# JaronTu/Multimodal_MVD_Seg

Hardware: AMD Instinct MI355X
Metric: train-step samples/sec on 4-modality 128^3 patches (PlainConvUNet 3d_fullres, fp32) (higher is better)
Workload: dtype f32; 1 GPU; BASELINE configs[1]: PlainConvUNet 3d_fullres 6 stages 31.2M params, 4x128x128x128 patch, 5 classes, fp32, DC+CE deep supervision, SGD-Nesterov+clip; per_gpu_batch=2, global_batch=2, parallelism=dp1, step_launch=one hipGraph replay per step (captured after 3 eager steps)

## Files before the change

include/mvdseg_hip.h:

```cpp
#ifndef MVDSEG_HIP_H
#define MVDSEG_HIP_H
#include <stddef.h>
#include <stdint.h>

#ifdef __cplusplus
extern "C" {
#endif

#define MVD_VERSION 100
#define MVD_MAX_TAPS 27

int mvd_version(void);
const char *mvd_last_error(void);
int mvd_has_mfma(void);
int mvd_set_conv_engine(int mode);
int mvd_set_wino_min_items(long n);

int mvd_pack_weight(const float *w, float *wf, float *wb, int K, int C, int T, int transposed, void *stream);

size_t mvd_conv_fwd_workspace_bytes(int N, long out_voxels, int K);
int mvd_conv3d_fwd(const float *x1, int C1, const float *x2, int C2, const float *wf, const float *bias, float *y,
                   int N, int D, int H, int W, int K, const int ksize[3], const int stride[3], void *ws,
                   size_t ws_bytes, void *stream);
int mvd_conv3d_dgrad(const float *dy, const float *wb, float *dx1, int C1, float *dx2, int C2, int N, int D, int H,
// ... 1 lines not shown
int mvd_conv_wino_applicable(int N, int D, int H, int W, int C1, int C2, int K, const int ksize[3], const int stride[3]);
size_t mvd_wino_weight_elems(int C, int K);
int mvd_wino_mode(void);
int mvd_pack_weight_wino(const float *w, float *uf, float *ub, int K, int C, void *stream);
int mvd_pack_weights_batch(int n, const float *const *w, float *const *wf, float *const *wb, float *const *uf,
                           float *const *ub, const int *K, const int *C, const int *T, const int *transposed,
                           void *stream);
int mvd_conv3d_fwd_wino(const float *x1, int C1, const float *x2, int C2, const float *wf, const float *uf,
                        const float *bias, float *y, int N, int D, int H, int W, int K, const int ksize[3],
                        const int stride[3], void *ws, size_t ws_bytes, void *stream);
size_t mvd_conv_stats_tiles(int D, int H, int W);
int mvd_conv3d_fwd_wino_stats(const float *x1, int C1, const float *x2, int C2, const float *wf, const float *uf,
                              const float *bias, float *y, float *stats, int *stats_done, int N, int D, int H, int W,
                              int K, const int ksize[3], const int stride[3], void *ws, size_t ws_bytes, void *stream);
int mvd_conv3d_dgrad_wino(const float *dy, const float *wb, const float *ub, float *dx1, int C1, float *dx2, int C2, int N,
                          int D, int H, int W, int K, const int ksize[3], const int stride[3], void *ws, size_t ws_bytes,
                          void *stream);
int mvd_set_wino3_min_items(long n);
int mvd_conv_wino3_applicable(int N, int D, int H, int W, int C1, int C2, int K, const int ksize[3], const int stride[3]);
size_t mvd_wino3_weight_elems(int C, int K);
int mvd_pack_weight_wino3(const float *w, float *vf, float *vb, int K, int C, void *stream);
int mvd_pack_weights_batch3(int n, const float *const *w, float *const *wf, float *const *wb, float *const *uf,
                            float *const *ub, float *const *vf, float *const *vb, const int *K, const int *C,
                            const int *T, const int *transposed, void *stream);
int mvd_conv3d_fwd_wino3(const float *x1, int C1, const float *x2, int C2, const float *wf, const float *vf,
                         const float *bias, float *y, int N, int D, int H, int W, int K, const int ksize[3],
                         const int stride[3], void *ws, size_t ws_bytes, void *stream);
int mvd_conv3d_fwd_wino3_stats(const float *x1, int C1, const float *x2, int C2, const float *wf, const float *vf,
                               const float *bias, float *y, float *stats, int *stats_done, int N, int D, int H, int W,
                               int K, const int ksize[3], const int stride[3], void *ws, size_t ws_bytes, void *stream);
int mvd_conv3d_dgrad_wino3(const float *dy, const float *wb, const float *vb, float *dx1, int C1, float *dx2, int C2,
                           int N, int D, int H, int W, int K, const int ksize[3], const int stride[3], void *ws,
                           size_t ws_bytes, void *stream);
size_t mvd_conv3d_wgrad_workspace_bytes(int C, int K, int T, int N, int Do, int Ho, int Wo);
int mvd_conv3d_wgrad(const float *x1, int C1, const float *x2, int C2, const float *dy, float *dw, float *dbias,
                     int N, int D, int H, int W, int K, const int ksize[3], const int stride[3], void *ws,
                     size_t ws_bytes, void *stream);

int mvd_convT3d_fwd(const float *x, const float *wf, const float *bias, float *y, int N, int D, int H, int W, int C,
                    int K, const int stride[3], void *ws, size_t ws_bytes, void *stream);
int mvd_convT3d_dgrad(const float *dy, const float *wb, float *dx, int N, int D, int H, int W, int C, int K,
                      const int stride[3], void *ws, size_t ws_bytes, void *stream);
size_t mvd_convT3d_wgrad_workspace_bytes(int C, int K, int T, int N, int D, int H, int W);
int mvd_convT3d_wgrad(const float *x, const float *dy, float *dw, float *dbias, int N, int D, int H, int W, int C,
                      int K, const int stride[3], void *ws, size_t ws_bytes, void *stream);

int mvd_pack_weight_bf16(const float *w, uint16_t *wf, uint16_t *wb, int K, int C, int T, int transposed, void *stream);
int mvd_pack_weights_bf16_batch(int n, const float *const *w, uint16_t *const *wf, uint16_t *const *wb, const int *K,
                                const int *C, const int *T, const int *transposed, void *stream);
int mvd_conv3d_fwd_bf16(const uint16_t *x1, int C1, const uint16_t *x2, int C2, const uint16_t *wf, const float *bias,
                        uint16_t *y, int N, int D, int H, int W, int K, const int ksize[3], const int stride[3],
                        void *ws, size_t ws_bytes, void *stream);
int mvd_conv3d_dgrad_bf16(const uint16_t *dy, const uint16_t *wb, uint16_t *dx1, int C1, uint16_t *dx2, int C2, int N,
                          int D, int H, int W, int K, const int ksize[3], const int stride[3], void *ws, size_t ws_bytes,
                          void *stream);
int mvd_convT3d_fwd_bf16(const uint16_t *x, const uint16_t *wf, const float *bias, uint16_t *y, int N, int D, int H, int W,
                         int C, int K, const int stride[3], void *ws, size_t ws_bytes, void *stream);
int mvd_convT3d_dgrad_bf16(const uint16_t *dy, const uint16_t *wb, uint16_t *dx, int N, int D, int H, int W, int C, int K,
                           const int stride[3], void *ws, size_t ws_bytes, void *stream);
int mvd_conv3d_wgrad_bf16(const uint16_t *x1, int C1, const uint16_t *x2, int C2, const uint16_t *dy, float *dw,
                          float *dbias, int N, int D, int H, int W, int K, const int ksize[3], const int stride[3],
                          void *ws, size_t ws_bytes, void *stream);
int mvd_convT3d_wgrad_bf16(const uint16_t *x, const uint16_t *dy, float *dw, float *dbias, int N, int D, int H, int W,
                           int C, int K, const int stride[3], void *ws, size_t ws_bytes, void *stream);
int mvd_conv3d_fwd_bf16_stats_tiles(int N, int D, int H, int W, int C1, int C2, int K, const int ksize[3],
                                    const int stride[3]);
// ... 157 lines not shown
```

multimodal_mvd_seg_amd/_lib.py:

```python
import ctypes
import os
from ctypes import c_float, c_int, c_long, c_size_t, c_void_p

_HERE = os.path.dirname(os.path.abspath(__file__))
LIB_PATH = os.path.join(_HERE, "libmvdseg_hip.so")

_P = c_void_p
_I3 = ctypes.c_int * 3

SIGNATURES = {
    "mvd_version": (c_int, []),
    "mvd_last_error": (ctypes.c_char_p, []),
    "mvd_has_mfma": (c_int, []),
    "mvd_set_conv_engine": (c_int, [c_int]),
    "mvd_set_wino_min_items": (c_int, [c_long]),
    "mvd_pack_weight": (c_int, [_P, _P, _P, c_int, c_int, c_int, c_int, _P]),
    "mvd_conv_fwd_workspace_bytes": (c_size_t, [c_int, c_long, c_int]),
    "mvd_conv3d_fwd": (c_int, [_P, c_int, _P, c_int, _P, _P, _P, c_int, c_int, c_int, c_int, c_int, _I3, _I3, _P,
                               c_size_t, _P]),
    "mvd_conv3d_dgrad": (c_int, [_P, _P, _P, c_int, _P, c_int, c_int, c_int, c_int, c_int, c_int, _I3, _I3, _P,
                                 c_size_t, _P]),
    "mvd_conv3d_wgrad_workspace_bytes": (c_size_t, [c_int, c_int, c_int, c_int, c_int, c_int, c_int]),
    "mvd_conv3d_wgrad": (c_int, [_P, c_int, _P, c_int, _P, _P, _P, c_int, c_int, c_int, c_int, c_int, _I3, _I3, _P,
                                 c_size_t, _P]),
    "mvd_convT3d_fwd": (c_int, [_P, _P, _P, _P, c_int, c_int, c_int, c_int, c_int, c_int, _I3, _P, c_size_t, _P]),
    "mvd_convT3d_dgrad": (c_int, [_P, _P, _P, c_int, c_int, c_int, c_int, c_int, c_int, _I3, _P, c_size_t, _P]),
    "mvd_convT3d_wgrad_workspace_bytes": (c_size_t, [c_int, c_int, c_int, c_int, c_int, c_int, c_int]),
    "mvd_convT3d_wgrad": (c_int, [_P, _P, _P, _P, c_int, c_int, c_int, c_int, c_int, c_int, _I3, _P, c_size_t, _P]),
    "mvd_conv_wino_applicable": (c_int, [c_int, c_int, c_int, c_int, c_int, c_int, c_int, _I3, _I3]),
    "mvd_wino_mode": (c_int, []),
    "mvd_wino_weight_elems": (c_size_t, [c_int, c_int]),
    "mvd_pack_weight_wino": (c_int, [_P, _P, _P, c_int, c_int, _P]),
    "mvd_pack_weights_batch": (c_int, [c_int] + [_P] * 9 + [_P]),
    "mvd_conv3d_fwd_wino": (c_int, [_P, c_int, _P, c_int, _P, _P, _P, _P, c_int, c_int, c_int, c_int, c_int, _I3, _I3, _P,
                                    c_size_t, _P]),
    "mvd_conv_stats_tiles": (c_size_t, [c_int, c_int, c_int]),
    "mvd_conv3d_fwd_wino_stats": (c_int, [_P, c_int, _P, c_int, _P, _P, _P, _P, _P, _P, c_int, c_int, c_int, c_int, c_int,
                                          _I3, _I3, _P, c_size_t, _P]),
    "mvd_conv3d_dgrad_wino": (c_int, [_P, _P, _P, _P, c_int, _P, c_int, c_int, c_int, c_int, c_int, c_int, _I3, _I3, _P,
                                      c_size_t, _P]),
    "mvd_set_wino3_min_items": (c_int, [c_long]),
    "mvd_conv_wino3_applicable": (c_int, [c_int, c_int, c_int, c_int, c_int, c_int, c_int, _I3, _I3]),
    "mvd_wino3_weight_elems": (c_size_t, [c_int, c_int]),
    "mvd_pack_weight_wino3": (c_int, [_P, _P, _P, c_int, c_int, _P]),
    "mvd_pack_weights_batch3": (c_int, [c_int] + [_P] * 11 + [_P]),
    "mvd_conv3d_fwd_wino3": (c_int, [_P, c_int, _P, c_int, _P, _P, _P, _P, c_int, c_int, c_int, c_int, c_int, _I3, _I3, _P,
                                     c_size_t, _P]),
    "mvd_conv3d_fwd_wino3_stats": (c_int, [_P, c_int, _P, c_int, _P, _P, _P, _P, _P, _P, c_int, c_int, c_int, c_int, c_int,
                                           _I3, _I3, _P, c_size_t, _P]),
    "mvd_conv3d_dgrad_wino3": (c_int, [_P, _P, _P, _P, c_int, _P, c_int, c_int, c_int, c_int, c_int, c_int, _I3, _I3, _P,
                                       c_size_t, _P]),
    "mvd_conv3d_wgrad_bf16": (c_int, [_P, c_int, _P, c_int, _P, _P, _P, c_int, c_int, c_int, c_int, c_int, _I3, _I3, _P,
                                      c_size_t, _P]),
    "mvd_convT3d_wgrad_bf16": (c_int, [_P, _P, _P, _P, c_int, c_int, c_int, c_int, c_int, c_int, _I3, _P, c_size_t,
                                       _P]),
    "mvd_instnorm_lrelu_fwd_prestats": (c_int, [_P, _P, c_long, _P, _P, _P, _P, _P, c_int, c_long, c_int, c_float, c_float,
                                                _P, c_size_t, _P]),
    "mvd_conv3d_fwd_bf16_stats_tiles": (c_int, [c_int, c_int, c_int, c_int, c_int, c_int, c_int, _I3, _I3]),
    "mvd_set_bf16_zmarch_kernel": (c_int, [c_int]),
    "mvd_set_bf16_wgrad_kernel": (c_int, [c_int]),
    "mvd_conv3d_dgrad_acc_ok": (c_int, [c_int, c_int, c_int, c_int, c_int, c_int, c_int, _I3, _I3]),
    "mvd_conv3d_dgrad_acc": (c_int, [_P, _P, _P, c_int, c_int, c_int, c_int, c_int, c_int, _I3, _I3, _P]),
    "mvd_conv3d_dgrad_bf16_acc": (c_int, [_P, _P, _P, c_int, c_int, c_int, c_int, c_int, c_int, _I3, _I3, _P, c_size_t, _P]),
    "mvd_conv3d_fwd_bf16_prologue_ok": (c_int, [c_int, c_int, c_int, c_int, c_int, c_int, c_int, _I3, _I3]),
    "mvd_conv3d_wgrad_bf16_prologue_ok": (c_int, [c_int, c_int, c_int, c_int, c_int, c_int, c_int, _I3, _I3]),
    "mvd_conv3d_wgrad_bf16_fused": (c_int, [_P, c_int, _P, _P, _P, c_int, c_int, c_int, c_int, c_int, _I3, _I3, _P, _P, c_float,
                                            _P, c_size_t, _P]),
    "mvd_instnorm_stats_bf16": (c_int, [_P, c_int, _P, _P, _P, _P, _P, _P, c_int, c_long, c_int, c_float, _P, c_size_t, _P]),
    "mvd_conv3d_fwd_bf16_fused": (c_int, [_P, c_int, _P, c_int, _P, _P, _P, c_int, c_int, c_int, c_int, c_int, _I3, _I3, _P,
                                          _P, c_float, _P, _P, _P, c_size_t, _P]),
    "mvd_instnorm_finalize_tiles": (c_int, [_P, c_long, _P, _P, _P, _P, _P, _P, c_int, c_long, c_int, c_float, _P]),
    "mvd_instnorm_lrelu_apply_bf16": (c_int, [_P, _P, _P, _P, c_int, c_long, c_int, c_float, _P]),
    "mvd_instnorm_lrelu_fwd_bf16": (c_int, [_P, c_int, _P, _P, _P, _P, _P, c_int, c_long, c_int, c_float, c_float, _P,
                                            c_size_t, _P]),
    "mvd_instnorm_lrelu_bwd_bf16": (c_int, [_P, c_int, _P, _P, _P, _P, _P, _P, _P, _P, c_int, c_long, c_int, c_float, _P,
                                            c_size_t, _P]),
    "mvd_seghead_fwd_bf16": (c_int, [_P, _P, _P, _P, c_int, c_long, c_int, c_int, _P]),
    "mvd_seghead_bwd_bf16": (c_int, [_P, _P, _P, _P, _P, _P, c_int, c_long, c_int, c_int, c_int, _P, c_size_t, _P]),
    "mvd_seghead_bf16_fused_ok": (c_int, [c_int, c_long, c_int, c_int]),
    "mvd_seghead_fwd_fused": (c_int, [_P, _P, _P, _P, _P, c_float, _P, _P, _P, c_int, c_long, c_int, c_int, _P]),
    "mvd_seghead_bwd_fused": (c_int, [_P, _P, _P, _P, _P, c_float, _P, _P, _P, _P, _P, c_int, c_long, c_int, c_int, c_int, _P,
                                      c_size_t, _P]),
    "mvd_instnorm_stats_from_tiles": (c_int, [_P, c_long, _P, _P, c_int, c_long, c_int, c_float, _P, c_size_t, _P]),
    "mvd_seghead_fwd_bf16_fused": (c_int, [_P, _P, _P, c_float, _P, _P, _P, c_int, c_long, c_int, c_int, _P]),
# ... 111 lines not shown
```

multimodal_mvd_seg_amd/csrc/conv.hip:

```cpp
#include "common.h"
#include "conv_geom.h"

namespace mvd {

static int g_engine_mode = 0;
#define g_wino_off (wino_mode() == 0)
static const int g_transp_off = getenv("MVD_TRANSP") ? (atoi(getenv("MVD_TRANSP")) == 0) : 0;
static long g_wino_min_items = getenv("MVD_WINO_MIN") ? atol(getenv("MVD_WINO_MIN")) : 256;
static const long kWino3MinItemsDefault = 128;
static long g_wino3_min_items = getenv("MVD_WINO3_MIN") ? atol(getenv("MVD_WINO3_MIN")) : kWino3MinItemsDefault;
static long wino3_items(int D, int H, int W, int K) { return (long)((D + 3) / 4) * ((H + 7) / 8) * ((W + 7) / 8) * (K / 32); }

__global__ void k_fwd_scalar(FwdGeom g, const float *__restrict__ a1, const float *__restrict__ a2,
                             const float *__restrict__ w, const float *__restrict__ bias, float *__restrict__ y1,
                             float *__restrict__ y2) {
    const int K = g.K1 + g.K2, C = g.C1 + g.C2;
    const int CK = wl_ck(C);
    const long total = (long)g.N * g.Do * g.Ho * g.Wo * K;
    for (long idx = (long)blockIdx.x * blockDim.x + threadIdx.x; idx < total; idx += (long)gridDim.x * blockDim.x) {
        int k = (int)(idx % K);
        long r = idx / K;
        int ow = (int)(r % g.Wo);
        r /= g.Wo;
        int oh = (int)(r % g.Ho);
// ... 562 lines not shown
                            const int st[3]) {
    memset(&g, 0, sizeof(g));
    g.N = N;
    g.Di = D; g.Hi = H; g.Wi = W;
    g.Do = out_dim(D, ks[0], st[0]); g.Ho = out_dim(H, ks[1], st[1]); g.Wo = out_dim(W, ks[2], st[2]);
    g.Db = g.Do; g.Hb = g.Ho; g.Wb = g.Wo;
    g.C1 = C1; g.C2 = C2; g.K = K;
    int t = 0;
    for (int a = 0; a < ks[0]; a++)
        for (int b = 0; b < ks[1]; b++)
            for (int c = 0; c < ks[2]; c++) {
                g.off[t][0] = a - (ks[0] - 1) / 2;
                g.off[t][1] = b - (ks[1] - 1) / 2;
                g.off[t][2] = c - (ks[2] - 1) / 2;
                g.wt[t] = t;
                t++;
            }
    g.ntaps = g.T = t;
    for (int a = 0; a < 3; a++) {
        g.sa[a] = st[a];
        g.sb[a] = 1;
    }
    g.transposed_out = 0;
}

size_t mvd_conv3d_wgrad_workspace_bytes(int C, int K, int T, int N, int Do, int Ho, int Wo) {
    WgradGeom g;
    memset(&g, 0, sizeof(g));
    g.N = N; g.Do = Do; g.Ho = Ho; g.Wo = Wo; g.C1 = C; g.C2 = 0; g.K = K; g.ntaps = g.T = T;
    size_t a = max_sz(wgrad_scalar_ws(g), wgrad_mfma_ws(g));
    return max_sz(a, colsum_ws((long)N * Do * Ho * Wo, K));
}

int mvd_conv3d_wgrad(const float *x1, int C1, const float *x2, int C2, const float *dy, float *dw, float *dbias, int N,
                     int D, int H, int W, int K, const int ksize[3], const int stride[3], void *ws, size_t ws_bytes,
                     void *stream) {
    MVD_REQUIRE(x1 && dy && dw && ws && C1 > 0 && C2 >= 0 && (C2 == 0 || x2), "conv3d_wgrad: null pointer / bad channels");
    MVD_REQUIRE(N > 0 && D > 0 && H > 0 && W > 0 && K > 0, "conv3d_wgrad: bad shape");
    if (check_ks(ksize, stride, "conv3d_wgrad")) return 2;
    WgradGeom g;
    conv_wgrad_geom(g, N, D, H, W, C1, C2, K, ksize, stride);
    MVD_REQUIRE(ws_bytes >= mvd_conv3d_wgrad_workspace_bytes(C1 + C2, K, g.T, N, g.Do, g.Ho, g.Wo),
                "conv3d_wgrad: workspace too small");
    hipStream_t s = as_stream(stream);
    int dbias_done = 0;
    int r = run_wgrad(g, x1, x2, dy, dw, ws, ws_bytes, s, dbias, &dbias_done);
    if (r) return r;
    if (dbias && !dbias_done) return colsum(dy, dbias, (long)N * g.Do * g.Ho * g.Wo, K, ws, s);
    return 0;
}

int mvd_convT3d_fwd(const float *x, const float *wf, const float *bias, float *y, int N, int D, int H, int W, int C, int K,
                    const int stride[3], void *ws, size_t ws_bytes, void *stream) {
    MVD_REQUIRE(x && wf && y && N > 0 && D > 0 && H > 0 && W > 0 && C > 0 && K > 0, "convT3d_fwd: bad arguments");
    for (int a = 0; a < 3; a++) MVD_REQUIRE(stride[a] == 1 || stride[a] == 2, "convT3d_fwd: stride must be 1 or 2");
    if (g_engine_mode == 0 && !g_transp_off) {
        int r = convT_fwd_direct(x, wf, bias, y, N, D, H, W, C, K, stride, as_stream(stream));
        if (r >= 0) return r;
    }
    for (int pd = 0; pd < stride[0]; pd++)
        for (int ph = 0; ph < stride[1]; ph++)
            for (int pw = 0; pw < stride[2]; pw++) {
                FwdGeom g;
                memset(&g, 0, sizeof(g));
                g.N = N;
                g.Di = g.Do = D; g.Hi = g.Ho = H; g.Wi = g.Wo = W;
// ... 414 lines not shown
```

multimodal_mvd_seg_amd/csrc/conv_geom.h:

```cpp
#pragma once
#include <stdint.h>

namespace mvd {

__host__ __device__ inline int wl_ck(int C) {
    return (C % 32 == 0) ? 32 : ((C % 8 == 0) ? 8 : ((C % 4 == 0) ? 4 : 0));
}
__host__ __device__ inline size_t widx(int CK, int T, int C, int K, int t, int c, int k) {
    if (CK == 0) return ((size_t)t * C + c) * K + k;
    const int hh = CK / 2;
    const int cc = c / CK, r = c % CK;
    return ((((size_t)cc * T + t) * 2 + r / hh) * K + k) * hh + (r % hh);
}

struct FwdGeom {
    int N;
    int T;
    int Di, Hi, Wi;
    int Do, Ho, Wo;
    int Dy, Hy, Wy;
    int C1, C2, K1, K2;
    int ntaps;
    int sa[3], so[3], oo[3];
    int8_t off[27][3];
// ... 24 lines not shown
int wgrad_scalar(const WgradGeom &g, const float *a1, const float *a2, const float *b, float *dw, void *ws,
                 size_t ws_bytes, hipStream_t s);
size_t wgrad_mfma_ws(const WgradGeom &g);
int wgrad_mfma(const WgradGeom &g, const float *a1, const float *a2, const float *b, float *dw, void *ws, size_t ws_bytes,
               hipStream_t s, bool bf16_in = false, float *dbias = nullptr, int *dbias_done = nullptr);

int fwd_wino(const FwdGeom &g, const float *a1, const float *a2, const float *u, const float *bias, float *y1, float *y2,
             hipStream_t s, float *stats = nullptr, int *stats_done = nullptr);
int pack_weight_wino(const float *w, float *uf, float *ub, int K, int C, hipStream_t s);
int fwd_wino3(const FwdGeom &g, const float *a1, const float *a2, const float *u, const float *bias, float *y1, float *y2,
              hipStream_t s, float *stats = nullptr, int *stats_done = nullptr);
int pack_weight_wino3(const float *w, float *uf, float *ub, int K, int C, hipStream_t s);
int wino3_enabled();
int dgrad32s(int N, int D, int H, int W, int C, int K, int Do, int Ho, int Wo, const float *dy, const float *wb, float *dx,
             hipStream_t s, int accumulate = 0);
int dgrad16s(int N, int D, int H, int W, int C, int K, int Do, int Ho, int Wo, const unsigned short *dy, const unsigned short *wb,
             unsigned short *dx, hipStream_t s, int accumulate = 0);
int launch_fwd16ys(const FwdGeom &g, const unsigned short *a1, const unsigned short *a2, const unsigned short *w, const float *bias,
                   unsigned short *y1, unsigned short *y2, hipStream_t s, int ncu);
int wgrad16z(const WgradGeom &g, const unsigned short *a1, const unsigned short *a2, const unsigned short *b, void *ws,
             size_t ws_bytes, bool want_bias, int *nsplit_out, float **pbias_out, hipStream_t s, const float *in_scale = nullptr,
             const float *in_shift = nullptr, float slope = 0.f);
int wgrad16z_run(const WgradGeom &g, const unsigned short *a1, const unsigned short *a2, const unsigned short *b, float *dw, void *ws,
                 size_t ws_bytes, hipStream_t s, float *dbias, int *dbias_done, const float *in_scale, const float *in_shift,
                 float slope);
bool wgrad16z_prologue_ok(const WgradGeom &g);
int wgrad16zs(const WgradGeom &g, const unsigned short *a1, const unsigned short *a2, const unsigned short *b, void *ws,
              size_t ws_bytes, int *nsplit_out, hipStream_t s);
void wgrad16z_enable(int on);
int pack_weights_batch(int n, const float *const *w, float *const *wf, float *const *wb, float *const *uf, float *const *ub,
                       const int *K, const int *C, const int *T, const int *transposed, hipStream_t s,
                       float *const *vf = nullptr, float *const *vb = nullptr);
int wino_mode();
size_t wino_weight_elems(int C, int K);

int convT_fwd_direct(const float *x, const float *wf, const float *bias, float *y, int N, int D, int H, int W, int C, int K,
                     const int st[3], hipStream_t s);
int convT_dgrad_direct(const float *dy, const float *wb, float *dx, int N, int D, int H, int W, int C, int K,
                       const int st[3], hipStream_t s);

int convT_fwd_direct16(const unsigned short *x, const unsigned short *wf, const float *bias, unsigned short *y, int N, int D,
                       int H, int W, int C, int K, const int st[3], hipStream_t s);
int convT_dgrad_direct16(const unsigned short *dy, const unsigned short *wb, unsigned short *dx, int N, int D, int H, int W,
                         int C, int K, const int st[3], hipStream_t s);

struct Fwd16Fuse {
    float *tile_stats = nullptr;
    int *ntiles = nullptr;
    const float *in_scale = nullptr, *in_shift = nullptr;
    float slope = 0.01f;
};
int fwd_bf16(const FwdGeom &g, const unsigned short *a1, const unsigned short *a2, const unsigned short *w,
             const float *bias, unsigned short *y1, unsigned short *y2, void *ws, size_t ws_bytes, hipStream_t s,
             const Fwd16Fuse *fuse = nullptr);
int fwd16y_enabled();
void fwd16y_enable(int on);
int launch_fwd16y(const FwdGeom &g, const unsigned short *a1, const unsigned short *a2, const unsigned short *w,
                  const float *bias, unsigned short *y1, unsigned short *y2, hipStream_t s, const Fwd16Fuse *fuse, int ncu,
                  int *stats_tiles_only);
int fwd_bf16_stats_tiles(const FwdGeom &g);
int fwd_bf16_prologue_ok(const FwdGeom &g);
int pack_weight16(const float *w, unsigned short *wf, unsigned short *wb, int K, int C, int T, int transposed,
                  hipStream_t s);
int pack_weights16_batch(int n, const float *const *w, unsigned short *const *wf, unsigned short *const *wb, const int *K,
                         const int *C, const int *T, const int *transposed, hipStream_t s);

// ... 2 lines not shown
```

multimodal_mvd_seg_amd/csrc/conv_mfma.hip:

```cpp
#include <stdlib.h>
#include <type_traits>

#include "common.h"
#include "conv_geom.h"

namespace mvd {

typedef float f32x16 __attribute__((ext_vector_type(16)));

struct FwdTile {
    int ED, EH, EW, nslots;
    int min_off[3];
    int ntd, nth, ntw;
    int K;
    int toff[27];
    int dbg;
};

__device__ __forceinline__ void store_tile32(const FwdGeom &g, const f32x16 &acc, float bv, int n, int od, int ohb, int ow0,
                                             int k, int hh, int S, int split, int Ktot, float *__restrict__ part,
                                             float *__restrict__ y1, float *__restrict__ y2) {
    const int owl = ow0 + 4 * hh;
    if (S > 1) {
        float *pl = part + (size_t)(4 * hh) * Ktot + k;
// ... 1755 lines not shown
        for (int r = 0; r < 16; r++) {
            const int row = (r & 3) + 8 * (r >> 2) + 4 * h;
            po[(size_t)(c0 + row) * K + k0 + i] = acc[j][r];
        }
    }
    if (A == 0 && B0 == 0 && GZ0 == 0 && pbias != nullptr && cb == 0) pbias[((size_t)split * 2 + h) * K + k0 + i] = bsum;
}

__global__ __launch_bounds__(1024) void k_dbias_reduce(const float *__restrict__ pbias, float *__restrict__ dbias, int K,
                                                       int nrows) {
    __shared__ double red[16][64];
    const int e = threadIdx.x & 63, q = threadIdx.x >> 6;
    const int k = blockIdx.x * 64 + e;
    double s = 0;
    if (k < K) {
        int r = q;
        for (; r + 48 < nrows; r += 64) {
            const float v0 = pbias[(size_t)r * K + k], v1 = pbias[(size_t)(r + 16) * K + k];
            const float v2 = pbias[(size_t)(r + 32) * K + k], v3 = pbias[(size_t)(r + 48) * K + k];
            s += (double)v0;
            s += (double)v1;
            s += (double)v2;
            s += (double)v3;
        }
        for (; r < nrows; r += 16) s += (double)pbias[(size_t)r * K + k];
    }
    red[q][e] = s;
    __syncthreads();
    if (q != 0 || k >= K) return;
    double t = 0;
#pragma unroll
    for (int j = 0; j < 16; j++) t += red[j][e];
    dbias[k] = (float)t;
}

template <int NA, int NB>
__global__ __launch_bounds__(256, 1) void k_wgrad_wino2(const WgradGeom g, const WgTile tg, const float *__restrict__ a1,
                                                        const float *__restrict__ a2, const float *__restrict__ b,
                                                        float *__restrict__ partial, float *__restrict__ pbias) {
    extern __shared__ __attribute__((aligned(16))) float lds[];
    float *As = lds;
    float *Bs = lds + (size_t)NA * 1024;
    const int wave = __builtin_amdgcn_readfirstlane(threadIdx.x >> 6);
    if (wave == 0) wgrad_wino2_body<0, 0, 4, 256, NA, NB>(g, tg, a1, a2, b, partial, pbias, As, Bs);
    else if (wave == 1) wgrad_wino2_body<1, 0, 4, 256, NA, NB>(g, tg, a1, a2, b, partial, pbias, As, Bs);
    else if (wave == 2) wgrad_wino2_body<2, 0, 4, 256, NA, NB>(g, tg, a1, a2, b, partial, pbias, As, Bs);
    else wgrad_wino2_body<3, 0, 4, 256, NA, NB>(g, tg, a1, a2, b, partial, pbias, As, Bs);
}

template <int NA8, int NB8>
__global__ __launch_bounds__(512, 2) void k_wgrad_wino2w8(const WgradGeom g, const WgTile tg, const float *__restrict__ a1,
                                                          const float *__restrict__ a2, const float *__restrict__ b,
                                                          float *__restrict__ partial, float *__restrict__ pbias) {
    extern __shared__ __attribute__((aligned(16))) float lds[];
    float *As = lds;
    float *Bs = lds + (size_t)NA8 * 2048;
    const int wave = __builtin_amdgcn_readfirstlane(threadIdx.x >> 6);
#define MVD_W8(AA, BB) wgrad_wino2_body<AA, BB, 2, 512, NA8, NB8>(g, tg, a1, a2, b, partial, pbias, As, Bs)
    switch (wave) {
        case 0: MVD_W8(0, 0); break;
        case 1: MVD_W8(0, 2); break;
        case 2: MVD_W8(1, 0); break;
        case 3: MVD_W8(1, 2); break;
        case 4: MVD_W8(2, 0); break;
        case 5: MVD_W8(2, 2); break;
        case 6: MVD_W8(3, 0); break;
// ... 626 lines not shown

static void launch_wgrad_reduce_f(unsigned blocks, hipStream_t s, const WgradGeom &g, const float *partial, float *dw, int nsplit,
                                  const float *pbias, float *dbias, int nrows, int wblocks) {
    static const int g16 = getenv("MVD_WGRAD_REDUCE_G16") ? atoi(getenv("MVD_WGRAD_REDUCE_G16")) : 1;
    if (g16 && nsplit >= 64)
        hipLaunchKernelGGL(k_wgrad_reduce_f<16>, dim3(blocks), dim3(1024), 0, s, g, partial, dw, nsplit, pbias, dbias, nrows, wblocks);
    else
        hipLaunchKernelGGL(k_wgrad_reduce_f<4>, dim3(blocks), dim3(256), 0, s, g, partial, dw, nsplit, pbias, dbias, nrows, wblocks);
}

static int wgrad_max_split(const WgradGeom &g, int per_cu = 2) {
    const int C = g.C1 + g.C2;
    const int ncb = (C + 31) / 32, nkb = (g.K + 31) / 32;
    long ns = 256L * per_cu / ((long)ncb * nkb);
    if (ns < 1) ns = 1;
    const long per = (long)g.ntaps * C * g.K * 4;
    long cap = (256L << 20) / per;
    if (cap < 1) cap = 1;
    if (ns > cap) ns = cap;
    return (int)ns;
}

static bool wgrad_mfma_ok(const WgradGeom &g) {
    const int C = g.C1 + g.C2;
    if (g.ntaps < 1 || g.ntaps > 27) return false;
    if (g.C1 % 4 != 0 || g.C2 % 4 != 0 || g.K % 4 != 0) return false;
    if (g.C2 > 0 && g.C1 % 32 != 0) return false;
    if (C < 4 || g.K < 4) return false;
    return true;
}

size_t wgrad_mfma_ws(const WgradGeom &g) {
    if (!wgrad_mfma_ok(g)) return 0;
    return (size_t)wgrad_max_split(g) * (g.ntaps * (size_t)(g.C1 + g.C2) + 2) * g.K * sizeof(float) + 256;
}

int wgrad16z_run(const WgradGeom &g, const unsigned short *a1, const unsigned short *a2, const unsigned short *b, float *dw, void *ws,
                 size_t ws_bytes, hipStream_t s, float *dbias, int *dbias_done, const float *in_scale, const float *in_shift,
                 float slope) {
    int nsplit_z = 0;
    float *pbias_z = nullptr;
    const int C = g.C1 + g.C2;
    const int rz = wgrad16z(g, a1, a2, b, ws, ws_bytes, dbias && dbias_done, &nsplit_z, &pbias_z, s, in_scale, in_shift, slope);
    if (rz != 0) return rz;
    float *partial_z = reinterpret_cast<float *>(ws);
    const int wblocks = (int)cdiv((long)27 * C * g.K, 64);
    if (pbias_z) {
        launch_wgrad_reduce_f((unsigned)(wblocks + cdiv(g.K, 64)), s, g, partial_z, dw, nsplit_z, pbias_z, dbias,
                           nsplit_z, wblocks);
        *dbias_done = 1;
    } else {
        launch_wgrad_reduce_f((unsigned)(wblocks), s, g, partial_z, dw, nsplit_z, (const float *)nullptr,
                           (float *)nullptr, 0, 0);
    }
    return check_launch("conv wgrad reduce (bf16 z-marching)");
}

int wgrad_mfma(const WgradGeom &g, const float *a1, const float *a2, const float *b, float *dw, void *ws, size_t ws_bytes,
               hipStream_t s, bool bf16_in, float *dbias, int *dbias_done) {
    if (dbias_done) *dbias_done = 0;
    if (!wgrad_mfma_ok(g)) return -1;
    if (((uintptr_t)a1 | (uintptr_t)a2 | (uintptr_t)b) & 15) return -1;
    if (bf16_in && (g.C1 % 32 != 0 || g.C2 % 32 != 0 || g.K % 32 != 0)) return -1;
    const int C = g.C1 + g.C2;
    if (bf16_in) {
        const int rz = wgrad16z_run(g, reinterpret_cast<const unsigned short *>(a1), reinterpret_cast<const unsigned short *>(a2),
                                    reinterpret_cast<const unsigned short *>(b), dw, ws, ws_bytes, s, dbias, dbias_done, nullptr,
// ... 171 lines not shown
            }
        } else if (cfg == 0) {
            if (sameB && tri) WG16T(7, 7, 2, 1, true);
            else if (sameB) WG16_TPW(7, 2, 1)
            else WG16_TPW(7, 2, 0)
        } else {
            if (sameA) WG16_TPW(1, 8, 2)
            else WG16_TPW(1, 8, 0)
        }
#undef WG16_TPW
#undef WG16
#undef WG16T
        if (check_launch("conv wgrad (bf16 mfma)")) return 1;
        const long per16 = (long)g.ntaps * C * g.K;
        const int wblocks = (int)cdiv(per16, 64);
        if (pbias16) {
            launch_wgrad_reduce_f((unsigned)(wblocks + cdiv(g.K, 64)), s, g, partial, dw, tg.nsplit, pbias16,
                               dbias, tg.nsplit, wblocks);
            *dbias_done = 1;
        } else {
            launch_wgrad_reduce_f((unsigned)(wblocks), s, g, partial, dw, tg.nsplit, (const float *)nullptr,
                               (float *)nullptr, 0, 0);
        }
        return check_launch("conv wgrad reduce (bf16 mfma)");
    }
    const int wino_off = wino_mode() == 0;
    if (!bf16_in && !wino_off && cfg == 0 && g.ntaps == 27 && g.T == 27 && !g.transposed_out && g.C1 % 32 == 0 &&
        g.C2 % 32 == 0 && g.K % 32 == 0 && tg.TD == 2) {
        bool plain = true;
        for (int a = 0; a < 3; a++) plain = plain && g.sa[a] == 1 && g.sb[a] == 1;
        for (int t = 0; t < 27 && plain; t++)
            plain = g.wt[t] == t && g.off[t][0] == t / 9 - 1 && g.off[t][1] == (t / 3) % 3 - 1 && g.off[t][2] == t % 3 - 1 &&
                    g.ob[t][0] == 0 && g.ob[t][1] == 0 && g.ob[t][2] == 0;
        const size_t need_w = (size_t)tg.nsplit * 36 * C * g.K * sizeof(float);
        if (plain && need_w <= ws_bytes) {
            const size_t need_m2 = (size_t)tg.nsplit * 48 * C * g.K * sizeof(float);
            const size_t need_w2 = need_m2 + (size_t)tg.nsplit * 2 * g.K * sizeof(float);
            if (wino_mode() == 2 && tg.TH == 8 && tg.TW == 8 && tg.EAh == 10 && tg.EAw == 10 && tg.EBh == 8 && tg.EBw == 8 &&
                need_w2 <= ws_bytes) {
                float *pbias = (dbias && dbias_done) ? partial + need_m2 / sizeof(float) : nullptr;
                static const int w8 = getenv("MVD_WGRAD_W8") ? atoi(getenv("MVD_WGRAD_W8")) : 12;
                static const int db12 = getenv("MVD_WGRAD_DB") ? atoi(getenv("MVD_WGRAD_DB")) : 1;
                auto kern2 = w8 == 12 ? (db12 ? k_wgrad_wino2w12<5, 2, true> : k_wgrad_wino2w12<5, 2, false>)
                                      : (w8 ? k_wgrad_wino2w8<7, 2> : k_wgrad_wino2<13, 4>);
                static PerDeviceFlag cfgd_w2;
                if (!cfgd_w2()) {
                    if (hipFuncSetAttribute(reinterpret_cast<const void *>(kern2), hipFuncAttributeMaxDynamicSharedMemorySize,
                                            (int)LDS_LIMIT) != hipSuccess) {
                        set_error("conv wgrad (winograd 2-D): cannot raise the dynamic LDS limit");
                        return 1;
                    }
                    cfgd_w2() = true;
                }
                hipLaunchKernelGGL(kern2, grid, dim3(w8 == 12 ? 768 : (w8 ? 512 : 256)),
                                   w8 == 12 ? (db12 ? (size_t)2 * (4 * 100 + 2 * 64) * 128 : (size_t)(5 + 2) * 12288)
                                            : (w8 ? (size_t)(7 + 2) * 8192 : (size_t)(13 + 4) * 4096), s, g,
                                   tg, a1, a2, b, partial, pbias);
                if (check_launch("conv wgrad (winograd 2-D)")) return 1;
                if (pbias) {
                    hipLaunchKernelGGL(k_dbias_reduce, dim3(cdiv(g.K, 64)), dim3(1024), 0, s, pbias, dbias, g.K, tg.nsplit * 2);
                    if (check_launch("conv wgrad dbias reduce")) return 1;
                    *dbias_done = 1;
                }
                hipLaunchKernelGGL(k_wgrad_reduce_wino2, dim3(cdiv((long)3 * C * g.K, 64)), dim3(1024), 0, s, partial, dw, C,
                                   g.K, tg.nsplit);
                return check_launch("conv wgrad reduce (winograd 2-D)");
// ... 73 lines not shown
```

Measured before the change: 58.26 samples/s.

## Add 3-D Winograd F(2,3) weight-gradient kernel for stride-1 3x3x3 convolutions

```diff
diff --git a/include/mvdseg_hip.h b/include/mvdseg_hip.h
--- a/include/mvdseg_hip.h
+++ b/include/mvdseg_hip.h
@@ -57,6 +57,10 @@
 int mvd_conv3d_dgrad_wino3(const float *dy, const float *wb, const float *vb, float *dx1, int C1, float *dx2, int C2,
                            int N, int D, int H, int W, int K, const int ksize[3], const int stride[3], void *ws,
                            size_t ws_bytes, void *stream);
+int mvd_set_wgrad_wino3_min_items(long n);
+int mvd_conv_wgrad_wino3_applicable(int N, int D, int H, int W, int C1, int C2, int K, const int ksize[3],
+                                    const int stride[3]);
+long mvd_wgrad_wino3_launches(void);
 size_t mvd_conv3d_wgrad_workspace_bytes(int C, int K, int T, int N, int Do, int Ho, int Wo);
 int mvd_conv3d_wgrad(const float *x1, int C1, const float *x2, int C2, const float *dy, float *dw, float *dbias,
                      int N, int D, int H, int W, int K, const int ksize[3], const int stride[3], void *ws,
diff --git a/multimodal_mvd_seg_amd/_lib.py b/multimodal_mvd_seg_amd/_lib.py
--- a/multimodal_mvd_seg_amd/_lib.py
+++ b/multimodal_mvd_seg_amd/_lib.py
@@ -50,6 +50,9 @@
                                            _I3, _I3, _P, c_size_t, _P]),
     "mvd_conv3d_dgrad_wino3": (c_int, [_P, _P, _P, _P, c_int, _P, c_int, c_int, c_int, c_int, c_int, c_int, _I3, _I3, _P,
                                        c_size_t, _P]),
+    "mvd_set_wgrad_wino3_min_items": (c_int, [c_long]),
+    "mvd_conv_wgrad_wino3_applicable": (c_int, [c_int, c_int, c_int, c_int, c_int, c_int, c_int, _I3, _I3]),
+    "mvd_wgrad_wino3_launches": (c_long, []),
     "mvd_conv3d_wgrad_bf16": (c_int, [_P, c_int, _P, c_int, _P, _P, _P, c_int, c_int, c_int, c_int, c_int, _I3, _I3, _P,
                                       c_size_t, _P]),
     "mvd_convT3d_wgrad_bf16": (c_int, [_P, _P, _P, _P, c_int, c_int, c_int, c_int, c_int, c_int, _I3, _P, c_size_t,
diff --git a/multimodal_mvd_seg_amd/csrc/conv.hip b/multimodal_mvd_seg_amd/csrc/conv.hip
--- a/multimodal_mvd_seg_amd/csrc/conv.hip
+++ b/multimodal_mvd_seg_amd/csrc/conv.hip
@@ -618,6 +618,23 @@
     return max_sz(a, colsum_ws((long)N * Do * Ho * Wo, K));
 }
 
+int mvd_set_wgrad_wino3_min_items(long n) {
+    set_wgrad_wino3_min_items(n);
+    return 0;
+}
+
+int mvd_conv_wgrad_wino3_applicable(int N, int D, int H, int W, int C1, int C2, int K, const int ksize[3],
+                                    const int stride[3]) {
+    if (N <= 0 || D <= 0 || H <= 0 || W <= 0 || C1 <= 0 || C2 < 0 || K <= 0 || !ksize || !stride) return 0;
+    for (int a = 0; a < 3; a++)
+        if (ksize[a] != 3 || stride[a] != 1) return 0;
+    WgradGeom g;
+    conv_wgrad_geom(g, N, D, H, W, C1, C2, K, ksize, stride);
+    return wgrad_wino3_selected(g) ? 1 : 0;
+}
+
+long mvd_wgrad_wino3_launches(void) { return wgrad_wino3_launches(); }
+
 int mvd_conv3d_wgrad(const float *x1, int C1, const float *x2, int C2, const float *dy, float *dw, float *dbias, int N,
                      int D, int H, int W, int K, const int ksize[3], const int stride[3], void *ws, size_t ws_bytes,
                      void *stream) {
diff --git a/multimodal_mvd_seg_amd/csrc/conv_geom.h b/multimodal_mvd_seg_amd/csrc/conv_geom.h
--- a/multimodal_mvd_seg_amd/csrc/conv_geom.h
+++ b/multimodal_mvd_seg_amd/csrc/conv_geom.h
@@ -80,6 +80,14 @@
                        const int *K, const int *C, const int *T, const int *transposed, hipStream_t s,
                        float *const *vf = nullptr, float *const *vb = nullptr);
 int wino_mode();
+int wgrad_wino3(const WgradGeom &g, const float *a1, const float *a2, const float *b, float *dw, void *ws, size_t ws_bytes,
+                int nsplit, hipStream_t s, float *dbias, int *dbias_done);
+bool wgrad_wino3_selected(const WgradGeom &g);
+size_t wgrad_wino3_ws(int nsplit, int C, int K);
+int wgrad_wino3_enabled();
+void set_wgrad_wino3_min_items(long n);
+long wgrad_wino3_launches();
+int dbias_reduce(const float *pbias, float *dbias, int K, int nrows, hipStream_t s);
 size_t wino_weight_elems(int C, int K);
 
 int convT_fwd_direct(const float *x, const float *wf, const float *bias, float *y, int N, int D, int H, int W, int C, int K,
diff --git a/multimodal_mvd_seg_amd/csrc/conv_mfma.hip b/multimodal_mvd_seg_amd/csrc/conv_mfma.hip
--- a/multimodal_mvd_seg_amd/csrc/conv_mfma.hip
+++ b/multimodal_mvd_seg_amd/csrc/conv_mfma.hip
@@ -1811,6 +1811,11 @@
 #pragma unroll
     for (int j = 0; j < 16; j++) t += red[j][e];
     dbias[k] = (float)t;
+}
+
+int dbias_reduce(const float *pbias, float *dbias, int K, int nrows, hipStream_t s) {
+    hipLaunchKernelGGL(k_dbias_reduce, dim3(cdiv(K, 64)), dim3(1024), 0, s, pbias, dbias, K, nrows);
+    return check_launch("conv wgrad dbias reduce");
 }
 
 template <int NA, int NB>
@@ -2503,7 +2508,13 @@
 
 size_t wgrad_mfma_ws(const WgradGeom &g) {
     if (!wgrad_mfma_ok(g)) return 0;
-    return (size_t)wgrad_max_split(g) * (g.ntaps * (size_t)(g.C1 + g.C2) + 2) * g.K * sizeof(float) + 256;
+    size_t ws = (size_t)wgrad_max_split(g) * (g.ntaps * (size_t)(g.C1 + g.C2) + 2) * g.K * sizeof(float) + 256;
+    const int C = g.C1 + g.C2;
+    if (g.ntaps == 27 && C % 32 == 0 && g.K % 32 == 0) {
+        const size_t w3 = wgrad_wino3_ws(wgrad_max_split(g, 1), C, g.K) + 256;
+        if (w3 > ws) ws = w3;
+    }
+    return ws;
 }
 
 int wgrad16z_run(const WgradGeom &g, const unsigned short *a1, const unsigned short *a2, const unsigned short *b, float *dw, void *ws,
@@ -2741,6 +2752,10 @@
         for (int t = 0; t < 27 && plain; t++)
             plain = g.wt[t] == t && g.off[t][0] == t / 9 - 1 && g.off[t][1] == (t / 3) % 3 - 1 && g.off[t][2] == t % 3 - 1 &&
                     g.ob[t][0] == 0 && g.ob[t][1] == 0 && g.ob[t][2] == 0;
+        if (plain && wgrad_wino3_selected(g)) {
+            const int r3 = wgrad_wino3(g, a1, a2, b, dw, ws, ws_bytes, wgrad_max_split(g, 1), s, dbias, dbias_done);
+            if (r3 >= 0) return r3;
+        }
         const size_t need_w = (size_t)tg.nsplit * 36 * C * g.K * sizeof(float);
         if (plain && need_w <= ws_bytes) {
             const size_t need_m2 = (size_t)tg.nsplit * 48 * C * g.K * sizeof(float);
diff --git a/multimodal_mvd_seg_amd/csrc/conv_wgrad_wino3.hip b/multimodal_mvd_seg_amd/csrc/conv_wgrad_wino3.hip
--- /dev/null
+++ b/multimodal_mvd_seg_amd/csrc/conv_wgrad_wino3.hip
@@ -0,0 +1,401 @@
+#include "common.h"
+#include "conv_geom.h"
+
+namespace mvd {
+
+typedef float f32x16 __attribute__((ext_vector_type(16)));
+typedef float v2f __attribute__((ext_vector_type(2)));
+
+struct Wg3Tile {
+    int ntd, nth, ntw;
+    int ntiles, nsplit, nkb;
+};
+
+constexpr int W3_EA = 10, W3_EB = 8;
+constexpr int W3_ABYTES = 4 * W3_EA * W3_EA * 128, W3_BBYTES = 2 * W3_EB * W3_EB * 128;
+constexpr int W3_IMG = W3_ABYTES + W3_BBYTES;
+
+template <bool PAIR, int A>
+__device__ __forceinline__ void wgrad_wino3_body(const int pz, const WgradGeom &g, const Wg3Tile &tg,
+                                                 const float *__restrict__ a1, const float *__restrict__ a2,
+                                                 const float *__restrict__ b, float *__restrict__ partial,
+                                                 float *__restrict__ pbias, float *lds) {
+    constexpr int RA = A == 0 ? 0 : (A == 2 ? 2 : 1);
+    constexpr int RB = A == 0 ? 2 : (A == 1 ? 2 : (A == 2 ? 1 : 3));
+    const int tid = threadIdx.x, lane = tid & 63;
+    const int i = lane & 31, h = lane >> 5;
+    const int cb = blockIdx.y / tg.nkb, kb = blockIdx.y % tg.nkb;
+    const int split = blockIdx.x;
+    const int C = g.C1 + g.C2, K = g.K;
+
+    f32x16 acc[4];
+#pragma unroll
+    for (int j = 0; j < 4; j++)
+#pragma unroll
+        for (int r = 0; r < 16; r++) acc[j][r] = 0.f;
+
+    const int c0 = cb * 32, k0 = kb * 32;
+    const float *asrc;
+    int Cs, cofs;
+    if (c0 < g.C1) {
+        asrc = a1; Cs = g.C1; cofs = c0;
+    } else {
+        asrc = a2; Cs = g.C2; cofs = c0 - g.C1;
+    }
+    const int planeA = g.Hi * g.Wi * Cs;
+    const int zb = tid >> 9, yb = (tid >> 6) & 7, xb = (tid >> 3) & 7;
+    const int relB = ((zb * g.Hb + yb) * g.Wb + xb) * K + k0 + (tid & 7) * 4;
+
+    v2f ra[4];
+    float4 rb;
+    auto load_tile = [&](int tile, bool valid) {
+        unsigned r_ = (unsigned)(valid ? tile : 0);
+        const int tw_ = (int)(r_ % (unsigned)tg.ntw); r_ /= (unsigned)tg.ntw;
+        const int th_ = (int)(r_ % (unsigned)tg.nth); r_ /= (unsigned)tg.nth;
+        const int td_ = (int)(r_ % (unsigned)tg.ntd);
+        const int n = (int)(r_ / (unsigned)tg.ntd);
+        const int z0 = td_ * 2, y0 = th_ * 8, x0 = tw_ * 8;
+        const bool intA = z0 >= 1 && y0 >= 1 && x0 >= 1 && z0 + 3 <= g.Di && y0 - 1 + W3_EA <= g.Hi && x0 - 1 + W3_EA <= g.Wi;
+        const bool intB = z0 + 2 <= g.Db && y0 + W3_EB <= g.Hb && x0 + W3_EB <= g.Wb;
+        const float *baseA = asrc + ((((long)n * g.Di + (z0 - 1)) * g.Hi + (y0 - 1)) * g.Wi + (x0 - 1)) * (long)Cs;
+        const float *baseB = b + ((((long)n * g.Db + z0) * g.Hb + y0) * g.Wb + x0) * (long)K;
+        const __amdgpu_buffer_rsrc_t rA =
+            __builtin_amdgcn_make_buffer_rsrc(const_cast<float *>(baseA), 0, valid ? 0x7fffffff : 0, 0x00020000);
+        const __amdgpu_buffer_rsrc_t rB =
+            __builtin_amdgcn_make_buffer_rsrc(const_cast<float *>(baseB), 0, valid ? 0x7fffffff : 0, 0x00020000);
+        struct Ld {
+            __amdgpu_buffer_rsrc_t rA, rB;
+            bool intA, intB;
+            int z0, y0, x0;
+        };
+        return Ld{rA, rB, intA, intB, z0, y0, x0};
+    };
+    auto issue_a = [&](const auto &L, int ph) {
+        const int q = tid + 1024 * ph, slot = q >> 4;
+        const int ya = slot / W3_EA, xa = slot - ya * W3_EA;
+        const unsigned rel = (unsigned)((ya * g.Wi + xa) * Cs + cofs + (q & 15) * 2);
+#pragma unroll
+        for (int u = 0; u < 4; u++) {
+            unsigned o = q < 16 * W3_EA * W3_EA ? (rel + (unsigned)(u * planeA)) * 4u : 0xffffffffu;
+            if (!L.intA) {
+                const int id = L.z0 - 1 + u, ih = L.y0 - 1 + ya, iw = L.x0 - 1 + xa;
+                const bool ok = id >= 0 && id < g.Di && ih >= 0 && ih < g.Hi && iw >= 0 && iw < g.Wi;
+                o = ok ? o : 0xffffffffu;
+            }
+            ra[u] = __builtin_bit_cast(v2f, __builtin_amdgcn_raw_buffer_load_b64(L.rA, (int)o, 0, 0));
+        }
+    };
+    auto issue_b = [&](const auto &L) {
+        unsigned o = (unsigned)relB * 4u;
+        if (!L.intB) {
+            const int id = L.z0 + zb, ih = L.y0 + yb, iw = L.x0 + xb;
+            o = (id < g.Db && ih < g.Hb && iw < g.Wb) ? o : 0xffffffffu;
+        }
+        rb = __builtin_bit_cast(float4, __builtin_amdgcn_raw_buffer_load_b128(L.rB, (int)o, 0, 0));
+    };
+    auto store_a = [&](int par, int ph) {
+        const int q = tid + 1024 * ph;
+        if (q >= 16 * W3_EA * W3_EA) return;
+        char *p = reinterpret_cast<char *>(lds) + par * W3_IMG + (q >> 4) * 128 + (q & 15) * 8;
+        constexpr int PL = W3_EA * W3_EA * 128;
+        *reinterpret_cast<v2f *>(p) = ra[0] - ra[2];
+        *reinterpret_cast<v2f *>(p + PL) = ra[1] + ra[2];
+        *reinterpret_cast<v2f *>(p + 2 * PL) = ra[2] - ra[1];
+        *reinterpret_cast<v2f *>(p + 3 * PL) = ra[1] - ra[3];
+    };
+    auto store_b = [&](int par) {
+        *reinterpret_cast<float4 *>(reinterpret_cast<char *>(lds) + par * W3_IMG + W3_ABYTES + tid * 16) = rb;
+    };
+
+    const char *img = reinterpret_cast<const char *>(lds);
+    const int abase = pz * (W3_EA * W3_EA * 128) + h * (2 * W3_EA * 128) + i * 4;
+    const int bbase = W3_ABYTES + h * (2 * W3_EB * 128) + i * 4;
+    const int zoff = pz == 3 ? W3_EB * W3_EB * 128 : 0;
+    const float esg = pz == 2 ? -1.f : 1.f;
+    auto fetch_col = [&](int s, int col, float &pa, float &pb) {
+        const int ad = abase + ((4 * s) * W3_EA + col) * 128;
+        pa = *reinterpret_cast<const float *>(img + ad + RA * W3_EA * 128);
+        pb = *reinterpret_cast<const float *>(img + ad + RB * W3_EA * 128);
+    };
+    auto rcomb = [&](float pa, float pb) { return A == 1 ? pa + pb : pa - pb; };
+    auto fetch_e = [&](int s, int wq, float (&e)[4], float (&f)[4]) {
+        const int ad = bbase + ((4 * s) * W3_EB + 2 * wq) * 128 + (PAIR ? 0 : zoff);
+        e[0] = *reinterpret_cast<const float *>(img + ad);
+        e[1] = *reinterpret_cast<const float *>(img + ad + 128);
+        e[2] = *reinterpret_cast<const float *>(img + ad + W3_EB * 128);
+        e[3] = *reinterpret_cast<const float *>(img + ad + W3_EB * 128 + 128);
+        if (PAIR) {
+            const int ad1 = ad + W3_EB * W3_EB * 128;
+            f[0] = *reinterpret_cast<const float *>(img + ad1);
+            f[1] = *reinterpret_cast<const float *>(img + ad1 + 128);
+            f[2] = *reinterpret_cast<const float *>(img + ad1 + W3_EB * 128);
+            f[3] = *reinterpret_cast<const float *>(img + ad1 + W3_EB * 128 + 128);
+        }
+    };
+    auto make_E = [&](float (&e)[4], const float (&f)[4], float (&E)[4]) {
+        if (PAIR) {
+#pragma unroll
+            for (int q = 0; q < 4; q++) e[q] = fmaf(esg, f[q], e[q]);
+        }
+        const float f0 = A == 0 ? e[0] : (A == 1 ? e[0] + e[2] : (A == 2 ? e[0] - e[2] : e[2]));
+        const float f1 = A == 0 ? e[1] : (A == 1 ? e[1] + e[3] : (A == 2 ? e[1] - e[3] : e[3]));
+        E[0] = f0; E[1] = f0 + f1; E[2] = f0 - f1; E[3] = f1;
+    };
+
+    float R[4];
+    float V[2][4];
+    float E[2][4];
+    const bool bias_wave = PAIR && A == 0 && pz == 1 && pbias != nullptr && cb == 0;
+    const float bflag = bias_wave ? 1.f : 0.f;
+    float bsum = 0.f;
+
+    int tile = split;
+    int par = 0;
+    {
+        const auto L = load_tile(tile, tile < tg.ntiles);
+#pragma unroll
+        for (int ph = 0; ph < 2; ph++) {
+            issue_a(L, ph);
+            store_a(0, ph);
+        }
+        issue_b(L);
+        store_b(0);
+        __syncthreads();
+    }
+    while (tile < tg.ntiles) {
+        const int next = tile + tg.nsplit;
+        const auto L = load_tile(next, next < tg.ntiles);
+        {
+            float e[4], f[4];
+            fetch_e(0, 0, e, f);
+#pragma unroll
+            for (int c = 0; c < 4; c++) {
+                float pa, pb;
+                fetch_col(0, c, pa, pb);
+                R[c] = rcomb(pa, pb);
+            }
+            make_E(e, f, E[0]);
+            if (PAIR && A == 0) bsum += bflag * ((e[0] + e[1]) + (e[2] + e[3]));
+            V[0][0] = R[0] - R[2];
+            V[0][1] = R[1] + R[2];
+            V[0][2] = R[2] - R[1];
+            V[0][3] = R[1] - R[3];
+        }
+        __builtin_amdgcn_sched_barrier(0);
+#pragma unroll
+        for (int t = 0; t < 8; t++) {
+            const int s = t >> 2, wq = t & 3, cur = t & 1, nxt = cur ^ 1;
+            const bool last = t == 7;
+            const int ns = wq == 3 ? s + 1 : s, nwq = wq == 3 ? 0 : wq + 1;
+            float pa[4], pb[4], e[4], f[4];
+#pragma unroll
+            for (int j = 0; j < 4; j++) {
+                acc[j] = __builtin_amdgcn_mfma_f32_32x32x2f32(V[cur][j], E[cur][j], acc[j], 0, 0, 0);
+                if (!last) {
+                    if (j == 0) fetch_e(ns, nwq, e, f);
+                    if (wq != 3) {
+                        if (j == 1) {
+                            fetch_col(ns, 2 * wq + 4, pa[0], pb[0]);
+                            fetch_col(ns, 2 * wq + 5, pa[1], pb[1]);
+                        }
+                    } else if (j == 1 || j == 2) {
+                        const int c2 = (j - 1) * 2;
+                        fetch_col(ns, c2, pa[c2], pb[c2]);
+                        fetch_col(ns, c2 + 1, pa[c2 + 1], pb[c2 + 1]);
+                    }
+                }
+                __builtin_amdgcn_sched_barrier(0);
+            }
+            if (!last) {
+                make_E(e, f, E[nxt]);
+                if (PAIR && A == 0) bsum += bflag * ((e[0] + e[1]) + (e[2] + e[3]));
+                if (wq != 3) {
+                    R[(2 * wq + 4) & 3] = rcomb(pa[0], pb[0]);
+                    R[(2 * wq + 5) & 3] = rcomb(pa[1], pb[1]);
+                } else {
+#pragma unroll
+                    for (int c = 0; c < 4; c++) R[c] = rcomb(pa[c], pb[c]);
+                }
+                const int x0 = 2 * nwq;
+                const float r0 = R[x0 & 3], r1 = R[(x0 + 1) & 3], r2 = R[(x0 + 2) & 3], r3 = R[(x0 + 3) & 3];
+                V[nxt][0] = r0 - r2;
+                V[nxt][1] = r1 + r2;
+                V[nxt][2] = r2 - r1;
+                V[nxt][3] = r1 - r3;
+            }
+            if (t == 0) issue_a(L, 0);
+            if (t == 1) issue_b(L);
+            if (t == 3) {
+                if (next < tg.ntiles) store_a(par ^ 1, 0);
+                issue_a(L, 1);
+            }
+            if (t == 6 && next < tg.ntiles) store_a(par ^ 1, 1);
+            if (t == 7 && next < tg.ntiles) store_b(par ^ 1);
+            __builtin_amdgcn_sched_barrier(0);
+        }
+        __syncthreads();
+        par ^= 1;
+        img = reinterpret_cast<const char *>(lds) + par * W3_IMG;
+        tile = next;
+    }
+#pragma unroll
+    for (int j = 0; j < 4; j++) {
+        float *po = partial + ((((size_t)split * 4 + pz) * 4 + A) * 4 + j) * C * K;
+#pragma unroll
+        for (int r = 0; r < 16; r++) {
+            const int row = (r & 3) + 8 * (r >> 2) + 4 * h;
+            po[(size_t)(c0 + row) * K + k0 + i] = acc[j][r];
+        }
+    }
+    if (bias_wave) pbias[((size_t)split * 2 + h) * K + k0 + i] = bsum;
+}
+
+__global__ __launch_bounds__(1024, 1) void k_wgrad_wino3(const WgradGeom g, const Wg3Tile tg, const float *__restrict__ a1,
+                                                         const float *__restrict__ a2, const float *__restrict__ b,
+                                                         float *__restrict__ partial, float *__restrict__ pbias) {
+    extern __shared__ __attribute__((aligned(16))) float lds[];
+    const int wave = __builtin_amdgcn_readfirstlane(threadIdx.x >> 6);
+    const int pz = wave >> 2;
+#define MVD_W3(PAIR, AA) wgrad_wino3_body<PAIR, AA>(pz, g, tg, a1, a2, b, partial, pbias, lds)
+    const bool pair = pz == 1 || pz == 2;
+    switch (wave & 3) {
+        case 0: if (pair) MVD_W3(true, 0); else MVD_W3(false, 0); break;
+        case 1: if (pair) MVD_W3(true, 1); else MVD_W3(false, 1); break;
+        case 2: if (pair) MVD_W3(true, 2); else MVD_W3(false, 2); break;
+        default: if (pair) MVD_W3(true, 3); else MVD_W3(false, 3); break;
+    }
+#undef MVD_W3
+}
+
+__global__ __launch_bounds__(1024) void k_wgrad_reduce_wino3(const float *__restrict__ partial, float *__restrict__ dw, int C,
+                                                             int K, int nsplit) {
+    __shared__ double r1[4][4][3][64];
+    __shared__ double r2[4][3][3][64];
+    const long CK = (long)C * K;
+    const long per = 64 * CK;
+    const int e = threadIdx.x & 63, w = threadIdx.x >> 6, pz = w >> 2, a = w & 3;
+    const long j = (long)blockIdx.x * 64 + e;
+    double m[4] = {0, 0, 0, 0};
+    if (j < CK) {
+        const float *src = partial + (size_t)w * 4 * CK + j;
+        int sp = 0;
+        for (; sp + 1 < nsplit; sp += 2) {
+            float v0[4], v1[4];
+#pragma unroll
+            for (int bq = 0; bq < 4; bq++) {
+                v0[bq] = src[(size_t)sp * per + (size_t)bq * CK];
+                v1[bq] = src[(size_t)(sp + 1) * per + (size_t)bq * CK];
+            }
+#pragma unroll
+            for (int bq = 0; bq < 4; bq++) {
+                m[bq] += (double)v0[bq];
+                m[bq] += (double)v1[bq];
+            }
+        }
+        if (sp < nsplit) {
+#pragma unroll
+            for (int bq = 0; bq < 4; bq++) m[bq] += (double)src[(size_t)sp * per + (size_t)bq * CK];
+        }
+    }
+    {
+        const bool neg = (pz == 3) != (a == 3);
+        const double m0 = neg ? -m[0] : m[0], m1 = neg ? -m[1] : m[1], m2 = neg ? -m[2] : m[2];
+        const double m3 = neg ? m[3] : -m[3];
+        r1[pz][a][0][e] = m0 + 0.5 * (m1 + m2);
+        r1[pz][a][1][e] = 0.5 * (m1 - m2);
+        r1[pz][a][2][e] = 0.5 * (m1 + m2) + m3;
+    }
+    __syncthreads();
+    if (w < 12) {
+        const int p2 = w / 3, l = w - p2 * 3;
+        const double q0 = r1[p2][0][l][e], q1 = r1[p2][1][l][e], q2 = r1[p2][2][l][e], q3 = r1[p2][3][l][e];
+        r2[p2][0][l][e] = q0 + 0.5 * (q1 + q2);
+        r2[p2][1][l][e] = 0.5 * (q1 - q2);
+        r2[p2][2][l][e] = 0.5 * (q1 + q2) + q3;
+    }
+    __syncthreads();
+    if (w >= 9 || j >= CK) return;
+    const int jj = w / 3, l = w - jj * 3;
+    const double q0 = r2[0][jj][l][e], q1 = r2[1][jj][l][e], q2 = r2[2][jj][l][e], q3 = r2[3][jj][l][e];
+    const int c = (int)(j / K), k = (int)(j - (long)c * K);
+    float *o = dw + ((size_t)k * C + c) * 27 + jj * 3 + l;
+    o[0 * 9] = (float)(q0 + 0.5 * (q1 + q2));
+    o[1 * 9] = (float)(0.5 * (q1 - q2));
+    o[2 * 9] = (float)(0.5 * (q1 + q2) + q3);
+}
+
+int wgrad_wino3_enabled() {
+    static int m = -1;
+    if (m < 0) m = getenv("MVD_WGRAD_WINO3") ? (atoi(getenv("MVD_WGRAD_WINO3")) != 0) : 1;
+    return m;
+}
+
+static const long kWgradWino3MinItemsDefault = 2048;
+static long g_wgrad_wino3_min_items =
+    getenv("MVD_WGRAD_WINO3_MIN") ? atol(getenv("MVD_WGRAD_WINO3_MIN")) : kWgradWino3MinItemsDefault;
+void set_wgrad_wino3_min_items(long n) { g_wgrad_wino3_min_items = n < 0 ? kWgradWino3MinItemsDefault : n; }
+
+bool wgrad_wino3_selected(const WgradGeom &g) {
+    if (!wgrad_wino3_enabled() || wino_mode() == 0) return false;
+    if (g.ntaps != 27 || g.T != 27 || g.transposed_out || g.C1 % 32 != 0 || g.C2 % 32 != 0 || g.K % 32 != 0) return false;
+    if (g.C1 + g.C2 < 32 || g.K < 32) return false;
+    for (int a = 0; a < 3; a++)
+        if (g.sa[a] != 1 || g.sb[a] != 1) return false;
+    for (int t = 0; t < 27; t++)
+        if (g.wt[t] != t || g.off[t][0] != t / 9 - 1 || g.off[t][1] != (t / 3) % 3 - 1 || g.off[t][2] != t % 3 - 1 ||
+            g.ob[t][0] != 0 || g.ob[t][1] != 0 || g.ob[t][2] != 0)
+            return false;
+    const long items = (long)((g.Do + 1) / 2) * ((g.Ho + 7) / 8) * ((g.Wo + 7) / 8) * ((g.C1 + g.C2) / 32) * (g.K / 32);
+    return items >= g_wgrad_wino3_min_items;
+}
+
+static long g_wgrad_wino3_launches = 0;
+long wgrad_wino3_launches() { return g_wgrad_wino3_launches; }
+
+size_t wgrad_wino3_ws(int nsplit, int C, int K) { return (size_t)nsplit * ((size_t)64 * C + 2) * K * sizeof(float); }
+
+int wgrad_wino3(const WgradGeom &g, const float *a1, const float *a2, const float *b, float *dw, void *ws, size_t ws_bytes,
+                int nsplit, hipStream_t s, float *dbias, int *dbias_done) {
+    const int C = g.C1 + g.C2;
+    Wg3Tile tg;
+    tg.ntd = (g.Do + 1) / 2;
+    tg.nth = (g.Ho + 7) / 8;
+    tg.ntw = (g.Wo + 7) / 8;
+    const long ntiles = (long)g.N * tg.ntd * tg.nth * tg.ntw;
+    if (ntiles > (1L << 30)) return -1;
+    tg.ntiles = (int)ntiles;
+    tg.nkb = g.K / 32;
+    const int ncb = C / 32;
+    if ((long)ncb * tg.nkb > 65535) return -1;
+    if (nsplit > ntiles) nsplit = (int)ntiles;
+    if (nsplit < 1) nsplit = 1;
+    tg.nsplit = nsplit;
+    if ((long)4 * g.Hi * g.Wi * g.C1 * 4 >= (1L << 31) || (long)4 * g.Hi * g.Wi * g.C2 * 4 >= (1L << 31) ||
+        (long)2 * g.Hb * g.Wb * g.K * 4 >= (1L << 31))
+        return -1;
+    if (wgrad_wino3_ws(nsplit, C, g.K) > ws_bytes) return -1;
+    float *partial = reinterpret_cast<float *>(ws);
+    const size_t nm = (size_t)nsplit * 64 * C * g.K;
+    float *pbias = (dbias && dbias_done) ? partial + nm : nullptr;
+    static PerDeviceFlag cfgd;
+    if (!cfgd()) {
+        if (hipFuncSetAttribute(reinterpret_cast<const void *>(k_wgrad_wino3), hipFuncAttributeMaxDynamicSharedMemorySize,
+                                2 * W3_IMG) != hipSuccess) {
+            set_error("conv wgrad (winograd 3-D): cannot raise the dynamic LDS limit");
+            return 1;
+        }
+        cfgd() = true;
+    }
+    hipLaunchKernelGGL(k_wgrad_wino3, dim3(nsplit, ncb * tg.nkb), dim3(1024), (size_t)2 * W3_IMG, s, g, tg, a1, a2, b,
+                       partial, pbias);
+    if (check_launch("conv wgrad (winograd 3-D)")) return 1;
+    g_wgrad_wino3_launches++;
+    if (pbias) {
+        if (dbias_reduce(pbias, dbias, g.K, nsplit * 2, s)) return 1;
+        *dbias_done = 1;
+    }
+    hipLaunchKernelGGL(k_wgrad_reduce_wino3, dim3(cdiv((long)C * g.K, 64)), dim3(1024), 0, s, partial, dw, C, g.K, nsplit);
+    return check_launch("conv wgrad reduce (winograd 3-D)");
+}
+
+}
```

Result: faster. 60.26 samples/s (median of 6 runs) (+3.4%).
